# salesforce/LayoutDETR

Measured on AMD Instinct MI355X. Metric: images/sec G+D fwd-bwd, 256x256 bg x9 elems, higher is better.
Workload: dtype f32

## Files before the change

layoutdetr_amd/csrc/p3_engine.hip:

```cpp
#include <cstdlib>
#include "ldetr_common.hpp"
#include "../../include/ldetr_hip.h"

namespace ldetr {

bool splitk_ws_alloc(long tiles, size_t partial_bytes, float** ws, int** counters);
void note_engine_launch(bool bf16_split_pipe);

typedef unsigned u32x4 __attribute__((ext_vector_type(4)));
typedef __attribute__((address_space(3))) void lds_void;

struct P3Epi {
    float alpha;
    const float* col_scale;
    const float* col_bias;
    const char* res_p3;
    const float* res_f32;
    const char* mask_p3;
    int relu;
    char* out_p3;
    float* out_f32;
};

struct P3NtParams {
    const char* A;
    const char* B;
    unsigned a_bytes, b_bytes;
    int M, N, Cin;
    int KH, KW, stride, pad;
    int H, W, OH, OW;
    int out_H, out_W, out_step, out_py, out_px;
    int tap_mode;
    int kh0, kw0, tstep, nty, ntx;
    int nkt;
    int splitk;
    float* ws; int* ws_count;
    int mtiles, ntiles, xm, xn;
    int nclass, nimg;
    P3Epi ep;
    int ngroups;
};

struct P3Group2 {
    const char* A2; const char* B2;
    P3Epi ep2;
};

__device__ __forceinline__ float bf_lo(unsigned w) { return __uint_as_float(w << 16); }
__device__ __forceinline__ float bf_hi(unsigned w) { return __uint_as_float(w & 0xffff0000u); }

__device__ __forceinline__ bool xcd_tile(int b, int mtiles, int ntiles, int xm, int xn, int& tm, int& tn) {
    const int x = b & 7, i = b >> 3, xi = x / xn, xj = x - xi * xn;
    const int mlo = xi * mtiles / xm, mhi = (xi + 1) * mtiles / xm, nlo = xj * ntiles / xn, nhi = (xj + 1) * ntiles / xn;
    const int cn = nhi - nlo;
    if (cn <= 0 || i >= (mhi - mlo) * cn) return false;
    tm = mlo + i / cn; tn = nlo + i - (i / cn) * cn;
    return true;
}

template <int WM, int WN, int TM, int TN, typename RowMap>
__device__ __forceinline__ void p3_wave_epilogue(const P3Epi& ep, float* Cs, const f32x16 (&acc)[TM][TN], int lane, int nbase, int N, RowMap rowmap) {
    constexpr int CP = WN + 4;
    const int cl = lane & 31, kl = lane >> 5;
#pragma unroll
    for (int i = 0; i < TM; i++)
#pragma unroll
        for (int j = 0; j < TN; j++)
#pragma unroll
            for (int r = 0; r < 16; r++)
                Cs[(i * 32 + (r & 3) + 8 * (r >> 2) + 4 * kl) * CP + j * 32 + cl] = acc[i][j][r];
    constexpr int CH = WN / 8;
    constexpr int RPI = 64 / CH;
    const int ch = lane % CH, rl0 = lane / CH;
    const int n = nbase + ch * 8;
    float cs[8], cb[8];
#pragma unroll
    for (int e = 0; e < 8; e++) { cs[e] = ep.alpha; cb[e] = 0.f; }
    if (n < N) {
        if (ep.col_scale) {
            const float4 s0 = *reinterpret_cast<const float4*>(ep.col_scale + n), s1 = *reinterpret_cast<const float4*>(ep.col_scale + n + 4);
            cs[0] *= s0.x; cs[1] *= s0.y; cs[2] *= s0.z; cs[3] *= s0.w; cs[4] *= s1.x; cs[5] *= s1.y; cs[6] *= s1.z; cs[7] *= s1.w;
        }
        if (ep.col_bias) {
            const float4 s0 = *reinterpret_cast<const float4*>(ep.col_bias + n), s1 = *reinterpret_cast<const float4*>(ep.col_bias + n + 4);
            cb[0] = s0.x; cb[1] = s0.y; cb[2] = s0.z; cb[3] = s0.w; cb[4] = s1.x; cb[5] = s1.y; cb[6] = s1.z; cb[7] = s1.w;
        }
    }
#pragma unroll 2
    for (int it = 0; it < WM / RPI; it++) {
        const int rl = it * RPI + rl0;
        const long orow = rowmap(rl);
        if (orow < 0 || n >= N) continue;
        const float4 v0 = *reinterpret_cast<const float4*>(Cs + rl * CP + ch * 8), v1 = *reinterpret_cast<const float4*>(Cs + rl * CP + ch * 8 + 4);
        float v[8] = {v0.x, v0.y, v0.z, v0.w, v1.x, v1.y, v1.z, v1.w};
#pragma unroll
        for (int e = 0; e < 8; e++) v[e] = v[e] * cs[e] + cb[e];
        const long goff = (orow * N + n) * 6;
        if (ep.res_p3) {
            const u32x4 h = *reinterpret_cast<const u32x4*>(ep.res_p3 + goff), md = *reinterpret_cast<const u32x4*>(ep.res_p3 + goff + 16),
                        lo = *reinterpret_cast<const u32x4*>(ep.res_p3 + goff + 32);
#pragma unroll
            for (int e = 0; e < 4; e++) {
                v[2 * e] += bf_lo(h[e]) + (bf_lo(md[e]) + bf_lo(lo[e]));
                v[2 * e + 1] += bf_hi(h[e]) + (bf_hi(md[e]) + bf_hi(lo[e]));
            }
        }
        if (ep.res_f32) {
            const float4 r0 = *reinterpret_cast<const float4*>(ep.res_f32 + orow * N + n), r1 = *reinterpret_cast<const float4*>(ep.res_f32 + orow * N + n + 4);
            v[0] += r0.x; v[1] += r0.y; v[2] += r0.z; v[3] += r0.w; v[4] += r1.x; v[5] += r1.y; v[6] += r1.z; v[7] += r1.w;
        }
        if (ep.relu) {
#pragma unroll
            for (int e = 0; e < 8; e++) v[e] = v[e] < 0.f ? 0.f : v[e];
        }
        if (ep.mask_p3) {
            const u32x4 h = *reinterpret_cast<const u32x4*>(ep.mask_p3 + goff);
#pragma unroll
            for (int e = 0; e < 4; e++) {
                if ((h[e] << 16) - 1u >= 0x7f800000u) v[2 * e] = 0.f;
                if ((h[e] & 0xffff0000u) - 1u >= 0x7f800000u) v[2 * e + 1] = 0.f;
            }
        }
        if (ep.out_f32) {
            *reinterpret_cast<float4*>(ep.out_f32 + orow * N + n) = make_float4(v[0], v[1], v[2], v[3]);
            *reinterpret_cast<float4*>(ep.out_f32 + orow * N + n + 4) = make_float4(v[4], v[5], v[6], v[7]);
        }
        if (ep.out_p3) {
            u32x4 h, md, lo;
#pragma unroll
            for (int e = 0; e < 4; e++) { unsigned a, b, c; split2_bf16_exact(v[2 * e], v[2 * e + 1], a, b, c); h[e] = a; md[e] = b; lo[e] = c; }
            *reinterpret_cast<u32x4*>(ep.out_p3 + goff) = h;
            *reinterpret_cast<u32x4*>(ep.out_p3 + goff + 16) = md;
            *reinterpret_cast<u32x4*>(ep.out_p3 + goff + 32) = lo;
        }
    }
}

template <int TM, int TN, int NT>
__device__ __forceinline__ bool p3_splitk_reduce(f32x16 (&acc)[TM][TN], float* ws, int* ws_count, long tile, int ks, int splitk, int tile_elems, int tid, int* flag) {
    float* slot0 = ws + tile * splitk * (long)tile_elems;
    float* mine = slot0 + (long)ks * tile_elems;
#pragma unroll
    for (int i = 0; i < TM; i++)
#pragma unroll
        for (int j = 0; j < TN; j++)
#pragma unroll
            for (int r = 0; r < 16; r++)
                __hip_atomic_store(mine + ((i * TN + j) * 16 + r) * NT + tid, acc[i][j][r], __ATOMIC_RELAXED, __HIP_MEMORY_SCOPE_AGENT);
    asm volatile("s_waitcnt vmcnt(0)" ::: "memory");
    __syncthreads();
    if (tid == 0) {
        const int old = atomicAdd(ws_count + tile, 1);
        const int last = old == splitk - 1;
        if (last) __hip_atomic_store(ws_count + tile, 0, __ATOMIC_RELAXED, __HIP_MEMORY_SCOPE_AGENT);
        *flag = last;
    }
    __syncthreads();
    const int last = *flag;
    __syncthreads();
    if (!last) return false;
#pragma unroll
    for (int i = 0; i < TM; i++)
#pragma unroll
        for (int j = 0; j < TN; j++)
#pragma unroll
            for (int r = 0; r < 16; r++) acc[i][j][r] = 0.f;
    for (int sl = 0; sl < splitk; sl++) {
        const float* src = slot0 + (long)sl * tile_elems;
#pragma unroll
        for (int i = 0; i < TM; i++)
#pragma unroll
            for (int j = 0; j < TN; j++)
#pragma unroll
                for (int r = 0; r < 16; r++)
                    acc[i][j][r] += __hip_atomic_load(src + ((i * TN + j) * 16 + r) * NT + tid, __ATOMIC_RELAXED, __HIP_MEMORY_SCOPE_AGENT);
    }
    return true;
}

template <int TM, int TN>
__device__ __forceinline__ bool p3_acc_non_finite(const f32x16 (&acc)[TM][TN]) {
    float chk = 0.f;
#pragma unroll
    for (int i = 0; i < TM; i++)
#pragma unroll
        for (int j = 0; j < TN; j++)
#pragma unroll
            for (int r = 0; r < 16; r++) chk = fmaf(acc[i][j][r], 0.f, chk);
    return __builtin_amdgcn_ballot_w64(chk != chk) != 0ull;
}

typedef unsigned int ld128_t __attribute__((__vector_size__(16)));

__device__ __forceinline__ void p3_load_group(const __amdgpu_buffer_rsrc_t rs, unsigned vo, int so, float (&v)[8]) {
    const ld128_t h = __builtin_amdgcn_raw_buffer_load_b128(rs, vo, so, 0), md = __builtin_amdgcn_raw_buffer_load_b128(rs, vo, so + 16, 0),
                  lo = __builtin_amdgcn_raw_buffer_load_b128(rs, vo, so + 32, 0);
#pragma unroll
    for (int e = 0; e < 4; e++) {
        v[2 * e] = bf_lo(h[e]) + (bf_lo(md[e]) + bf_lo(lo[e]));
        v[2 * e + 1] = bf_hi(h[e]) + (bf_hi(md[e]) + bf_hi(lo[e]));
    }
}

__device__ __forceinline__ float p3_load_elem(const __amdgpu_buffer_rsrc_t rs, unsigned row, int c) {
    const unsigned vo = row == 0x80000000u ? row : row + (unsigned)((c >> 3) * 48 + (c & 7) * 2);
    const unsigned h = __builtin_amdgcn_raw_buffer_load_b16(rs, vo, 0, 0), md = __builtin_amdgcn_raw_buffer_load_b16(rs, vo, 16, 0),
                   lo = __builtin_amdgcn_raw_buffer_load_b16(rs, vo, 32, 0);
    return bf_lo(h) + (bf_lo(md) + bf_lo(lo));
}

template <int WM, int WN, int TM, int TN, typename Dot>
__device__ __forceinline__ void p3_cold_tile(f32x16 (&acc)[TM][TN], float* img, int lane, Dot dot) {
    for (int e = lane; e < WM * WN; e += 64) {
        const int row = e / WN, col = e - row * WN;
        const float v = dot(row, col);
        const int i = row >> 5, rr = row & 31, j = col >> 5, cl = col & 31;
// ... 139 lines not shown
    const int rr = lane >> 2, pq = (lane & 3) ^ ((rr >> 2) & 3);
    const int ktpt = p.Cin >> 5;
    unsigned offA[RGA], vmA[RGA], offB[RGB];
#pragma unroll
    for (int i = 0; i < RGA; i++) {
        unsigned vm, off;
        p3_nt_row(p, m0 + (w * RGA + i) * 16 + rr, off, vm);
        offA[i] = (ONE && vm == 0u) ? 0x80000000u : off + pq * 16; vmA[i] = vm;
    }
#pragma unroll
    for (int i = 0; i < RGB; i++) {
        const int n = n0 + (w * RGB + i) * 16 + rr;
        offB[i] = n < p.N ? (unsigned)n * (unsigned)(p.KH * p.KW * p.Cin) * 6u + pq * 16 : 0x80000000u;
    }

    int tap = ONE ? 0 : kt0 / ktpt, cc = kt0 - tap * ktpt;

    const int frr = cl & 15, frg = cl >> 4;
    unsigned fo[2][3];
#pragma unroll
    for (int s = 0; s < 2; s++)
#pragma unroll
        for (int pl = 0; pl < 3; pl++) {
            const int e = 3 * (2 * s + kl) + pl;
            fo[s][pl] = (unsigned)((frg * 3 + (e >> 2)) * 1024 + frr * 64 + (((e & 3) ^ ((frr >> 2) & 3)) << 4));
        }
    const unsigned foA = (unsigned)(wm * (WM / 16) * 3 * 1024), foB = (unsigned)(A_BYTES + wn * (WN / 16) * 3 * 1024);

    f32x16 acc[TM][TN];
#pragma unroll
    for (int i = 0; i < TM; i++)
#pragma unroll
        for (int j = 0; j < TN; j++)
#pragma unroll
            for (int r = 0; r < 16; r++) acc[i][j][r] = 0.f;

    const int nloc = kt1 - kt0;
    ld128_t ra[PF][RGA * 3], rb[PF][RGB * 3];
#pragma unroll
    for (int d = 0; d < PF; d++) p3_load_tile<BM, BN, NW, ONE>(p, rsA, rsB, offA, vmA, offB, tap, cc, ktpt, d < nloc, ra[d], rb[d]);
    if (nloc > 0) p3_store_tile<BM, BN, NW>(p3_smem, w, lane, ra[0], rb[0]);
    __syncthreads();
    for (int it0 = 0; it0 < nloc; it0 += PF) {
#pragma unroll
        for (int d = 0; d < PF; d++) {
            const int it = it0 + d;
            p3_load_tile<BM, BN, NW, ONE>(p, rsA, rsB, offA, vmA, offB, tap, cc, ktpt, it + PF < nloc, ra[d], rb[d]);
            __builtin_amdgcn_sched_barrier(0);
            if (it < nloc) {
                const char* sb = p3_smem + (it % NST) * ST_BYTES;
#pragma unroll
                for (int s = 0; s < 2; s++) {
                    bf16x8_t a[TM][3], b[TN][3];
#pragma unroll
                    for (int i = 0; i < TM; i++)
#pragma unroll
                        for (int pl = 0; pl < 3; pl++)
                            a[i][pl] = *reinterpret_cast<const bf16x8_t*>(sb + foA + i * (2 * 3 * 1024) + fo[s][pl]);
#pragma unroll
                    for (int j = 0; j < TN; j++)
#pragma unroll
                        for (int pl = 0; pl < 3; pl++)
                            b[j][pl] = *reinterpret_cast<const bf16x8_t*>(sb + foB + j * (2 * 3 * 1024) + fo[s][pl]);
#pragma unroll
                    for (int i = 0; i < TM; i++)
#pragma unroll
                        for (int j = 0; j < TN; j++) {
                            acc[i][j] = __builtin_amdgcn_mfma_f32_32x32x16_bf16(a[i][1], b[j][1], acc[i][j], 0, 0, 0);
                            acc[i][j] = __builtin_amdgcn_mfma_f32_32x32x16_bf16(a[i][0], b[j][2], acc[i][j], 0, 0, 0);
                            acc[i][j] = __builtin_amdgcn_mfma_f32_32x32x16_bf16(a[i][2], b[j][0], acc[i][j], 0, 0, 0);
                            acc[i][j] = __builtin_amdgcn_mfma_f32_32x32x16_bf16(a[i][0], b[j][1], acc[i][j], 0, 0, 0);
                            acc[i][j] = __builtin_amdgcn_mfma_f32_32x32x16_bf16(a[i][1], b[j][0], acc[i][j], 0, 0, 0);
                            acc[i][j] = __builtin_amdgcn_mfma_f32_32x32x16_bf16(a[i][0], b[j][0], acc[i][j], 0, 0, 0);
                        }
                }
                if (NST == 1) __syncthreads();
                if (it + 1 < nloc) p3_store_tile<BM, BN, NW>(p3_smem + ((it + 1) % NST) * ST_BYTES, w, lane, ra[(d + 1) % PF], rb[(d + 1) % PF]);
                __syncthreads();
            }
        }
    }

    constexpr int CP = WN + 4;
    if (p3_acc_non_finite<TM, TN>(acc)) {
        p3_cold_tile<WM, WN, TM, TN>(acc, reinterpret_cast<float*>(p3_smem) + w * (WM * CP), lane, [&](int row, int col) -> float {
            unsigned off, vm;
            p3_nt_row(p, m0 + wm * WM + row, off, vm);
            const int n = n0 + wn * WN + col;
            const unsigned ob = n < p.N ? (unsigned)n * (unsigned)(p.KH * p.KW * p.Cin) * 6u : 0x80000000u;
            float s = 0.f;
            for (int kt = kt0; kt < kt1; kt++) {
                const int tp = kt / ktpt;
                int sA, sB;
                p3_nt_koff(p, tp, kt - tp * ktpt, sA, sB);
                const unsigned vo = ((vm >> tp) & 1u) ? off : 0x80000000u;
                for (int g = 0; g < 4; g++) {
                    float a[8], b[8];
                    p3_load_group(rsA, vo, sA + g * 48, a); p3_load_group(rsB, ob, sB + g * 48, b);
#pragma unroll
                    for (int e = 0; e < 8; e++) s = fmaf(a[e], b[e], s);
                }
            }
            return s;
        });
    }
    if (p.splitk > 1 && !p3_splitk_reduce<TM, TN, NT>(acc, p.ws, p.ws_count, ws_tile0 + t, ks, p.splitk, BM * BN, tid, reinterpret_cast<int*>(p3_smem))) return;
    const int ohw = p.OH * p.OW;
    p3_wave_epilogue<WM, WN, TM, TN>(p.ep, reinterpret_cast<float*>(p3_smem) + w * (WM * CP), acc, lane, n0 + wn * WN, p.N, [&](int rl) -> long {
        const int m = m0 + wm * WM + rl;
        if (m >= p.M) return -1;
        if (p.out_step == 1 && p.out_H == p.OH && p.out_W == p.OW) return m;
        const int nn = m / ohw, rem = m - nn * ohw, oy = rem / p.OW, ox = rem - oy * p.OW;
        return ((long)nn * p.out_H + (oy * p.out_step + p.out_py)) * p.out_W + (ox * p.out_step + p.out_px);
    });
}

template <int BM, int BN, int NW, int PF, int NST, bool ONE = false>
__global__ __launch_bounds__(NW * 64) void p3_nt_kernel(P3NtParams p, P3Group2 g2) { p3_nt_body<BM, BN, NW, PF, NST, true, ONE>(p, g2, blockIdx.x, blockIdx.y, blockIdx.z); }

struct P3C3Params {
    const char* X; const char* Wt;
    unsigned x_bytes, w_bytes;
    int N_img, H, W, Cin, Nout;
    int lgPW, lgPH, NP;
    int HWp, HPIX, NH, NG;
    int ppr, ppi;
    int flip;
    int ncc;
    int splitk; float* ws; int* ws_count;
    int mtiles, ntiles, xm, xn;
    P3Epi ep;
    int ngroups;
};

constexpr int C3_NGMAX = 13, C3_A_BYTES = C3_NGMAX * 3072, C3_B_BYTES = 4 * 3072, C3_LDS = C3_A_BYTES + 3 * C3_B_BYTES;

__device__ __forceinline__ void p3_c3_decode_tile_row(const P3C3Params& p, int tm, int r, int& n, int& y0, int& x0, int& py, int& px) {
    const int lgpp = p.lgPW + p.lgPH;
    const int sp = r >> lgpp, q = r & ((1 << lgpp) - 1);
    py = q >> p.lgPW; px = q & ((1 << p.lgPW) - 1);
    const int pid = tm * p.NP + sp;
    n = pid / p.ppi; const int prem = pid - n * p.ppi;
    const int pr = prem / p.ppr, pc = prem - pr * p.ppr;
    y0 = pr << p.lgPH; x0 = pc << p.lgPW;
}

template <int TAP>
__device__ __forceinline__ void p3_c3_tap(const P3C3Params& p, const __amdgpu_buffer_rsrc_t rsA, const __amdgpu_buffer_rsrc_t rsB, char* smem, int w, int lane,
                                          const unsigned (&offA)[4], unsigned offB, int cc, bool more_cc, bool more_tile,
                                          ld128_t (&ar)[12], ld128_t (&br)[3], const unsigned (&h0)[2], const unsigned (&ce)[2][3], const unsigned (&fo)[2][3],
                                          unsigned foB, f32x16 (&acc)[2][1]) {
    if (more_tile) {
        const int ntap = TAP == 8 ? 0 : TAP + 1, ncc = TAP == 8 ? cc + 1 : cc;
        const int sB = ntap * p.Cin * 6 + ncc * 192;
#pragma unroll
        for (int j = 0; j < 3; j++) br[j] = __builtin_amdgcn_raw_buffer_load_b128(rsB, offB, sB + j * 64, 0);
    }
    if (more_cc) {
#pragma unroll
        for (int q = TAP * 12 / 9; q < (TAP + 1) * 12 / 9; q++)
            ar[q] = __builtin_amdgcn_raw_buffer_load_b128(rsA, offA[q / 3], (cc + 1) * 192 + (q % 3) * 64, 0);
    }
    constexpr int ty = TAP / 3, tx = TAP % 3;
    const int dt = p.flip ? (2 - ty) * p.HWp + (2 - tx) : ty * p.HWp + tx;
    unsigned hb[2], sw[2];
#pragma unroll
    for (int i = 0; i < 2; i++) {
        const unsigned h = h0[i] + dt;
        hb[i] = (h >> 4) * 3072 + ((h & 15) << 6);
        sw[i] = ((h >> 2) & 3) << 4;
    }
    const char* sb = smem + C3_A_BYTES + (TAP % 3) * C3_B_BYTES + foB;
#pragma unroll
    for (int s2 = 0; s2 < 2; s2++) {
        bf16x8_t a[2][3], b[3];
#pragma unroll
        for (int i = 0; i < 2; i++)
#pragma unroll
            for (int pl = 0; pl < 3; pl++) a[i][pl] = *reinterpret_cast<const bf16x8_t*>(smem + hb[i] + (ce[s2][pl] ^ sw[i]));
#pragma unroll
        for (int pl = 0; pl < 3; pl++) b[pl] = *reinterpret_cast<const bf16x8_t*>(sb + fo[s2][pl]);
#pragma unroll
        for (int i = 0; i < 2; i++) {
            acc[i][0] = __builtin_amdgcn_mfma_f32_32x32x16_bf16(a[i][1], b[1], acc[i][0], 0, 0, 0);
            acc[i][0] = __builtin_amdgcn_mfma_f32_32x32x16_bf16(a[i][0], b[2], acc[i][0], 0, 0, 0);
            acc[i][0] = __builtin_amdgcn_mfma_f32_32x32x16_bf16(a[i][2], b[0], acc[i][0], 0, 0, 0);
            acc[i][0] = __builtin_amdgcn_mfma_f32_32x32x16_bf16(a[i][0], b[1], acc[i][0], 0, 0, 0);
            acc[i][0] = __builtin_amdgcn_mfma_f32_32x32x16_bf16(a[i][1], b[0], acc[i][0], 0, 0, 0);
            acc[i][0] = __builtin_amdgcn_mfma_f32_32x32x16_bf16(a[i][0], b[0], acc[i][0], 0, 0, 0);
        }
    }
    if (more_tile) {
        char* dst = smem + C3_A_BYTES + ((TAP + 1) % 3) * C3_B_BYTES + w * 3072 + lane * 16;
#pragma unroll
        for (int j = 0; j < 3; j++) *reinterpret_cast<ld128_t*>(dst + j * 1024) = br[j];
    }
    __syncthreads();
}

template <bool GROUPS>
__device__ __forceinline__ void p3_c3_body(P3C3Params p, const P3Group2& g2, const int bx, const int by, const int bz) {
    constexpr int BM = 128, BN = 64, NT = 256, WM = 64, WN = 32;
    if (GROUPS && p.ngroups > 1 && bz > 0) { p.X = g2.A2; p.Wt = g2.B2; p.ep = g2.ep2; }
    extern __shared__ __attribute__((aligned(1024))) char p3_smem[];
    const int tid = threadIdx.x, lane = tid & 63, w = __builtin_amdgcn_readfirstlane(tid >> 6), wm = w >> 1, wn = w & 1;
    const int cl = lane & 31, kl = lane >> 5;
    int tm, tn;
    if (!xcd_tile(bx, p.mtiles, p.ntiles, p.xm, p.xn, tm, tn)) return;
    const int t = tm * p.ntiles + tn;
    const int n0 = tn * BN;
    const int ks = by;
    const int per = (p.ncc + p.splitk - 1) / p.splitk;
    const int cc0 = ks * per, cc1 = min(p.ncc, cc0 + per);

    const __amdgpu_buffer_rsrc_t rsA = __builtin_amdgcn_make_buffer_rsrc(const_cast<char*>(p.X), 0, p.x_bytes, 0x00020000);
    const __amdgpu_buffer_rsrc_t rsB = __builtin_amdgcn_make_buffer_rsrc(const_cast<char*>(p.Wt), 0, p.w_bytes, 0x00020000);

    const int rr = lane >> 2, pq = (lane & 3) ^ ((rr >> 2) & 3);
    unsigned offA[4], offB;
#pragma unroll
    for (int i = 0; i < 4; i++) {
        const int h = (w + 4 * i) * 16 + rr;
        unsigned off = 0x80000000u;
        if (h < p.NH) {
            const int sp = h / p.HPIX, rem = h - sp * p.HPIX, hy = rem / p.HWp, hx = rem - hy * p.HWp;
            const int pid = tm * p.NP + sp;
            const int n = pid / p.ppi, prem = pid - n * p.ppi, pr = prem / p.ppr, pc = prem - pr * p.ppr;
            const int y = (pr << p.lgPH) + hy - 1, x = (pc << p.lgPW) + hx - 1;
            if (n < p.N_img && y >= 0 && y < p.H && x >= 0 && x < p.W) off = (unsigned)(((n * p.H + y) * p.W + x) * p.Cin) * 6u + pq * 16;
        }
        offA[i] = off;
    }
    {
        const int n = n0 + w * 16 + rr;
        offB = n < p.Nout ? (unsigned)n * (unsigned)(9 * p.Cin) * 6u + pq * 16 : 0x80000000u;
    }
    unsigned h0[2];
#pragma unroll
    for (int i = 0; i < 2; i++) {
        const int r = wm * WM + i * 32 + cl;
        const int lgpp = p.lgPW + p.lgPH;
        const int sp = r >> lgpp, q = r & ((1 << lgpp) - 1);
        h0[i] = (unsigned)(sp * p.HPIX + (q >> p.lgPW) * p.HWp + (q & ((1 << p.lgPW) - 1)));
    }
    const int frr = cl & 15, frg = cl >> 4;
    unsigned ce[2][3], fo[2][3];
#pragma unroll
    for (int s2 = 0; s2 < 2; s2++)
#pragma unroll
        for (int pl = 0; pl < 3; pl++) {
            const int e = 3 * (2 * s2 + kl) + pl;
            ce[s2][pl] = (unsigned)(((e >> 2) * 1024) | ((e & 3) << 4));
            fo[s2][pl] = (unsigned)((frg * 3 + (e >> 2)) * 1024 + frr * 64 + (((e & 3) ^ ((frr >> 2) & 3)) << 4));
        }
    const unsigned foB = (unsigned)(wn * 2 * 3072);

    f32x16 acc[2][1];
#pragma unroll
    for (int i = 0; i < 2; i++)
#pragma unroll
        for (int r = 0; r < 16; r++) acc[i][0][r] = 0.f;

    ld128_t ar[12], br[3];
    if (cc1 > cc0) {
#pragma unroll
        for (int q = 0; q < 12; q++) ar[q] = __builtin_amdgcn_raw_buffer_load_b128(rsA, offA[q / 3], cc0 * 192 + (q % 3) * 64, 0);
#pragma unroll
        for (int j = 0; j < 3; j++) br[j] = __builtin_amdgcn_raw_buffer_load_b128(rsB, offB, cc0 * 192 + j * 64, 0);
#pragma unroll
        for (int q = 0; q < 12; q++)
            if (w + 4 * (q / 3) < C3_NGMAX) *reinterpret_cast<ld128_t*>(p3_smem + ((w + 4 * (q / 3)) * 3 + (q % 3)) * 1024 + lane * 16) = ar[q];
#pragma unroll
        for (int j = 0; j < 3; j++) *reinterpret_cast<ld128_t*>(p3_smem + C3_A_BYTES + w * 3072 + j * 1024 + lane * 16) = br[j];
    }
    __syncthreads();
    for (int cc = cc0; cc < cc1; cc++) {
        const bool more_cc = cc + 1 < cc1;
#define C3_TAP(T_) p3_c3_tap<T_>(p, rsA, rsB, p3_smem, w, lane, offA, offB, cc, more_cc, (T_) < 8 || more_cc, ar, br, h0, ce, fo, foB, acc)
        C3_TAP(0); C3_TAP(1); C3_TAP(2); C3_TAP(3); C3_TAP(4); C3_TAP(5); C3_TAP(6); C3_TAP(7); C3_TAP(8);
#undef C3_TAP
        if (more_cc) {
#pragma unroll
            for (int q = 0; q < 12; q++)
                if (w + 4 * (q / 3) < C3_NGMAX) *reinterpret_cast<ld128_t*>(p3_smem + ((w + 4 * (q / 3)) * 3 + (q % 3)) * 1024 + lane * 16) = ar[q];
            __syncthreads();
        }
    }

    constexpr int CP = WN + 4;
    static_assert(4 * WM * CP * 4 <= C3_LDS, "epilogue staging does not fit");
    if (p3_acc_non_finite<2, 1>(acc)) {
        p3_cold_tile<WM, WN, 2, 1>(acc, reinterpret_cast<float*>(p3_smem) + w * (WM * CP), lane, [&](int row, int col) -> float {
            int n, y0, x0, py, px;
            p3_c3_decode_tile_row(p, tm, wm * WM + row, n, y0, x0, py, px);
            if (n >= p.N_img) return 0.f;
            const int y = y0 + py, x = x0 + px, no = n0 + wn * WN + col;
            const unsigned ob = no < p.Nout ? (unsigned)no * (unsigned)(9 * p.Cin) * 6u : 0x80000000u;
            float s = 0.f;
            for (int cc = cc0; cc < cc1; cc++)
                for (int tap = 0; tap < 9; tap++) {
                    const int ty = tap / 3, tx = tap - ty * 3;
                    const int sy = y + (p.flip ? 1 - ty : ty - 1), sx = x + (p.flip ? 1 - tx : tx - 1);
                    const unsigned vo = (sy >= 0 && sy < p.H && sx >= 0 && sx < p.W) ? (unsigned)(((n * p.H + sy) * p.W + sx) * p.Cin) * 6u : 0x80000000u;
                    for (int g = 0; g < 4; g++) {
                        float a[8], b[8];
                        p3_load_group(rsA, vo, cc * 192 + g * 48, a); p3_load_group(rsB, ob, tap * p.Cin * 6 + cc * 192 + g * 48, b);
#pragma unroll
                        for (int e = 0; e < 8; e++) s = fmaf(a[e], b[e], s);
                    }
                }
            return s;
        });
    }
    if (p.splitk > 1 && !p3_splitk_reduce<2, 1, NT>(acc, p.ws, p.ws_count, t + bz * p.mtiles * p.ntiles, ks, p.splitk, BM * BN, tid, reinterpret_cast<int*>(p3_smem))) return;
    p3_wave_epilogue<WM, WN, 2, 1>(p.ep, reinterpret_cast<float*>(p3_smem) + w * (WM * CP), acc, lane, n0 + wn * WN, p.Nout, [&](int rl) -> long {
        int n, y0, x0, py, px;
        p3_c3_decode_tile_row(p, tm, wm * WM + rl, n, y0, x0, py, px);
        if (n >= p.N_img) return -1;
        return ((long)n * p.H + (y0 + py)) * p.W + (x0 + px);
    });
}

__global__ __launch_bounds__(256, 2) void p3_c3_kernel(P3C3Params p, P3Group2 g2) { p3_c3_body<true>(p, g2, blockIdx.x, blockIdx.y, blockIdx.z); }

struct P3TnParams {
    const char* dY; const char* X;
    unsigned dy_bytes, x_bytes;
    int Cout, Cin, KH, KW, stride, pad;
    int H, W, OH, OW;
    int npix;
    float inv_ohw, inv_ow;
    int mtiles, ntiles, splitk;
    const float* row_scale;
    float alpha;
    float* dW;
};

__device__ __forceinline__ void fastdivmod(int x, int d, float invd, int& q, int& r) {
    q = (int)((float)x * invd);
    r = x - q * d;
    if (r >= d) { ++q; r -= d; }
    if (r < 0) { --q; r += d; }
}

typedef unsigned u32x2_t __attribute__((ext_vector_type(2)));
__device__ __forceinline__ u32x2_t tr_read(unsigned addr) {
    u32x2_t v;
    asm volatile("ds_read_b64_tr_b16 %0, %1" : "=v"(v) : "v"(addr) : "memory");
    return v;
}
__device__ __forceinline__ void tr_wait() { asm volatile("s_waitcnt lgkmcnt(0)" ::: "memory"); __builtin_amdgcn_sched_barrier(0); }
__device__ __forceinline__ bf16x8_t tr_join(u32x2_t lo, u32x2_t hi) {
    const u32x4 v = {lo[0], lo[1], hi[0], hi[1]};
    return __builtin_bit_cast(bf16x8_t, v);
}

template <int BM, int BN>
__device__ __forceinline__ void p3_tn_load(const P3TnParams& p, const __amdgpu_buffer_rsrc_t rsA, const __amdgpu_buffer_rsrc_t rsB, int w, int lane,
                                           int k0, int kend, int m0, int n0, int kh, int kw, ld128_t* ra, ld128_t* rb) {
    constexpr int UA = BM / 64, UB = BN / 64;
    const int rg = w & 1, rr = lane >> 2, pq = (lane & 3) ^ ((rr >> 2) & 3);
    const int pix = k0 + rg * 16 + rr;
    const bool inr = pix < kend;
    const unsigned offA = inr ? (unsigned)pix * (unsigned)p.Cout * 6u + pq * 16 : 0x80000000u;
#pragma unroll
    for (int i = 0; i < UA; i++) {
        const int cb = (w >> 1) * UA + i;
        const int sA = (m0 + cb * 32) * 6;
#pragma unroll
        for (int j = 0; j < 3; j++) ra[i * 3 + j] = __builtin_amdgcn_raw_buffer_load_b128(rsA, offA, sA + j * 64, 0);
    }
    unsigned offB = 0x80000000u;
    {
        int n, rem, oy, ox;
        fastdivmod(pix, p.OH * p.OW, p.inv_ohw, n, rem);
        fastdivmod(rem, p.OW, p.inv_ow, oy, ox);
        const int sy = oy * p.stride - p.pad + kh, sx = ox * p.stride - p.pad + kw;
        if (inr && sy >= 0 && sy < p.H && sx >= 0 && sx < p.W)
            offB = (unsigned)(((n * p.H + oy * p.stride) * p.W + ox * p.stride) * p.Cin) * 6u + pq * 16;
    }
    const int sBt = (kh * p.W + kw) * p.Cin * 6;
#pragma unroll
    for (int i = 0; i < UB; i++) {
        const int cb = (w >> 1) * UB + i;
        const int sB = sBt + (n0 + cb * 32) * 6;
#pragma unroll
        for (int j = 0; j < 3; j++) rb[i * 3 + j] = __builtin_amdgcn_raw_buffer_load_b128(rsB, offB, sB + j * 64, 0);
    }
}

template <int BM, int BN>
__device__ __forceinline__ void p3_tn_store(char* sb, int w, int lane, const ld128_t* ra, const ld128_t* rb) {
    constexpr int UA = BM / 64, UB = BN / 64, A_BYTES = BM * 192;
    const int rg = w & 1;
#pragma unroll
    for (int i = 0; i < UA; i++)
#pragma unroll
        for (int j = 0; j < 3; j++) *reinterpret_cast<ld128_t*>(sb + ((((w >> 1) * UA + i) * 2 + rg) * 3 + j) * 1024 + lane * 16) = ra[i * 3 + j];
#pragma unroll
    for (int i = 0; i < UB; i++)
// ... 215 lines not shown
#pragma unroll
        for (int e = 0; e < 4; e++) { unsigned a, b, c; split2_bf16_exact(v[2 * e], v[2 * e + 1], a, b, c); h[e] = a; md[e] = b; lo[e] = c; }
        char* d = dst + u * 48;
        *reinterpret_cast<u32x4*>(d) = h; *reinterpret_cast<u32x4*>(d + 16) = md; *reinterpret_cast<u32x4*>(d + 32) = lo;
    }
}

__global__ __launch_bounds__(256) void p3_weight_prep_kernel(const long long* __restrict__ table, int nconv) {
    int c = 0;
    while (c + 1 < nconv && (long long)blockIdx.x >= table[(c + 1) * 8 + 7]) ++c;
    const long long* row = table + c * 8;
    const float* w = reinterpret_cast<const float*>(row[0]);
    const float* sc = reinterpret_cast<const float*>(row[1]);
    char* df = reinterpret_cast<char*>(row[2]);
    char* db = reinterpret_cast<char*>(row[3]);
    const int O = (int)row[4], T = (int)row[5], I = (int)row[6];
    const long u = ((long)blockIdx.x - row[7]) * 256 + threadIdx.x;
    const long units = (long)O * T * I / 8;
    if (u >= units) return;
    if (df) {
        const float4 v0 = *reinterpret_cast<const float4*>(w + u * 8), v1 = *reinterpret_cast<const float4*>(w + u * 8 + 4);
        const float v[8] = {v0.x, v0.y, v0.z, v0.w, v1.x, v1.y, v1.z, v1.w};
        u32x4 h, md, lo;
#pragma unroll
        for (int e = 0; e < 4; e++) { unsigned a, b, cc; split2_bf16_exact(v[2 * e], v[2 * e + 1], a, b, cc); h[e] = a; md[e] = b; lo[e] = cc; }
        char* d = df + u * 48;
        *reinterpret_cast<u32x4*>(d) = h; *reinterpret_cast<u32x4*>(d + 16) = md; *reinterpret_cast<u32x4*>(d + 32) = lo;
    }
    if (db) {
        const int i = (int)(u % I); const long r = u / I; const int tp = (int)(r % T); const int g = (int)(r / T);
        float v[8];
#pragma unroll
        for (int e = 0; e < 8; e++) v[e] = w[((long)(g * 8 + e) * T + tp) * I + i] * (sc ? sc[g * 8 + e] : 1.f);
        u32x4 h, md, lo;
#pragma unroll
        for (int e = 0; e < 4; e++) { unsigned a, b, cc; split2_bf16_exact(v[2 * e], v[2 * e + 1], a, b, cc); h[e] = a; md[e] = b; lo[e] = cc; }
        char* d = db + (((long)i * T + tp) * (O / 8) + g) * 48;
        *reinterpret_cast<u32x4*>(d) = h; *reinterpret_cast<u32x4*>(d + 16) = md; *reinterpret_cast<u32x4*>(d + 32) = lo;
    }
}

static void choose_xcd_array(int mtiles, int ntiles, double a_bytes, double b_bytes, int& xm, int& xn, long& grid_x) {
    double best = -1.0; xm = 8; xn = 1;
    for (int n = 1; n <= 8; n *= 2) {
        const int m = 8 / n;
        if ((n > ntiles && n > 1) || (m > mtiles && m > 1)) continue;
        const double cost = a_bytes * n + b_bytes * m;
        if (best < 0 || cost < best) { best = cost; xm = m; xn = n; }
    }
    grid_x = 8L * cdiv(mtiles, xm) * cdiv(ntiles, xn);
}


struct RaisedPerDevice { bool on[64] = {}; };
static bool raise_lds(const void* kern, size_t lds, const char* what, RaisedPerDevice& raised) {
    if (lds <= 64 * 1024) return true;
    int dev = 0;
    if (hipGetDevice(&dev) != hipSuccess || dev < 0 || dev >= 64) dev = -1;
    if (dev >= 0 && raised.on[dev]) return true;
    if (hipFuncSetAttribute(kern, hipFuncAttributeMaxDynamicSharedMemorySize, (int)lds) != hipSuccess) {
        set_error("%s: cannot raise the dynamic LDS limit to %zu bytes", what, lds);
        return false;
    }
    if (dev >= 0) raised.on[dev] = true;
    return true;
}

struct P3LastLaunch { int kind, bm, bn, nw, splitk, xm, xn, ncls, tn_splitk; long grid; };
static thread_local P3LastLaunch t_last = {0, 0, 0, 0, 0, 0, 0, 0, 0, 0};

struct NtGrid { long gx; int sk, ncls; size_t lds; };

template <int BM, int BN, int NW, int NST>
static NtGrid plan_nt(P3NtParams& p, int sk) {
    p.mtiles = cdiv(p.M, BM); p.ntiles = cdiv(p.N, BN);
    NtGrid g; g.ncls = p.nclass > 1 ? p.nclass : (p.ngroups > 1 ? p.ngroups : 1);
    const long nt = (long)p.mtiles * p.ntiles;
    choose_xcd_array(p.mtiles, p.ntiles, (double)p.M * p.Cin * 6.0, (double)p.N * p.KH * p.KW * p.Cin * 6.0, p.xm, p.xn, g.gx);
    if (sk > p.nkt) sk = p.nkt;
    if (sk < 1) sk = 1;
    p.splitk = sk; p.ws = nullptr; p.ws_count = nullptr;
    if (sk > 1 && !splitk_ws_alloc(nt * g.ncls, (size_t)nt * g.ncls * sk * BM * BN * sizeof(float), &p.ws, &p.ws_count)) p.splitk = sk = 1;
    g.sk = sk;
    constexpr int WGN_ = (NW == 8 && BN >= 128) ? 4 : 2, WM_ = BM / (NW / WGN_), WN_ = BN / WGN_;
    constexpr size_t lds_loop = (size_t)NST * (BM + BN) * 192, lds_epi = (size_t)NW * WM_ * (WN_ + 4) * 4;
    g.lds = lds_loop > lds_epi ? lds_loop : lds_epi;
    return g;
}

static long slot_target(double flops, long dflt) {
    static const double small = 1.5 * 1e9;
    return (flops < small && dflt > 256) ? 256 : dflt;
}
static double nt_flops(const P3NtParams& p) { return 2.0 * p.M * p.N * p.nkt * 32.0 * (p.nclass > 1 ? p.nclass : 1); }
static double tn_flops(const P3TnParams& p) { return 2.0 * p.npix * p.Cout * (double)p.Cin * p.KH * p.KW; }

static int nt_splitk(const P3NtParams& p, int bm, int bn, long slots) {
    const long nt = (long)cdiv(p.M, bm) * cdiv(p.N, bn);
    int sk = 1;
    if (nt < slots * 3 / 4) { sk = (int)(slots / nt); if (sk > p.nkt / 4) sk = p.nkt / 4; if (sk > 16) sk = 16; if (sk < 1) sk = 1; }
    return sk;
}

static bool nt_is_plain_gemm(const P3NtParams& p) { return p.KH * p.KW == 1 && p.pad == 0 && p.nclass <= 1 && (p.tap_mode == 0 || p.stride == 1); }

template <int BM, int BN, int NW, int PF, int NST>
static int launch_nt_cfg(P3NtParams& p, const P3Group2& g2, int sk, hipStream_t st) {
    const NtGrid g = plan_nt<BM, BN, NW, NST>(p, sk);
    if constexpr (PF == 1 && NST == 1 && (BM == BN) && (NW == 4 ? BM == 64 : BM == 128)) {
        if (nt_is_plain_gemm(p)) {
            auto kern1 = p3_nt_kernel<BM, BN, NW, PF, NST, true>;
            static RaisedPerDevice raised1;
            if (!raise_lds(reinterpret_cast<const void*>(kern1), g.lds, "p3_nt", raised1)) return LDETR_ERR_LAUNCH;
            hipLaunchKernelGGL(kern1, dim3((unsigned)g.gx, g.sk, g.ncls), NW * 64, g.lds, st, p, g2);
            t_last = {1, BM, BN, NW, g.sk, p.xm, p.xn, g.ncls, 0, g.gx};
            note_engine_launch(true);
            return check_launch("p3_nt");
        }
    }
    auto kern = p3_nt_kernel<BM, BN, NW, PF, NST>;
    static RaisedPerDevice raised;
    if (!raise_lds(reinterpret_cast<const void*>(kern), g.lds, "p3_nt", raised)) return LDETR_ERR_LAUNCH;
    hipLaunchKernelGGL(kern, dim3((unsigned)g.gx, g.sk, g.ncls), NW * 64, g.lds, st, p, g2);
    t_last = {1, BM, BN, NW, g.sk, p.xm, p.xn, g.ncls, 0, g.gx};
    note_engine_launch(true);
    return check_launch("p3_nt");
}

static int launch_nt(P3NtParams& p, const P3Group2& g2, bool forward, hipStream_t st) {
    static const int force_tile = (int)knob("P3_TILE", 0);
    int cfg = 3;
    if (forward && p.nclass <= 1 && ((p.M >= 65536 && p.N >= 128) || (p.M >= 16384 && p.N >= 256 && p.nkt <= 16))) cfg = 1;
    if (force_tile) cfg = force_tile;
    const int bm = cfg == 3 ? 64 : 128, bn = (cfg == 1 || cfg == 4) ? 128 : 64;
    const int sk = nt_splitk(p, bm, bn, slot_target(nt_flops(p), (cfg == 2 || cfg == 3) ? 512 : 256));
    switch (cfg) {
        case 1: return launch_nt_cfg<128, 128, 8, 1, 1>(p, g2, sk, st);
        case 2: return launch_nt_cfg<128, 64, 4, 1, 1>(p, g2, sk, st);
        case 3: return launch_nt_cfg<64, 64, 4, 1, 1>(p, g2, sk, st);
        default: return launch_nt_cfg<128, 128, 4, 1, 1>(p, g2, sk, st);
    }
}

static bool c3_geometry(int N, int H, int W, P3C3Params& p) {
    auto lg = [](int v) { int l = 0; while ((1 << l) < v) ++l; return (1 << l) == v ? l : -1; };
    int PW = W < 16 ? W : 16;
    if (lg(PW) < 0 || W % PW) return false;
    int PH = 128 / PW; if (PH > H) PH = H;
    while (PH > 1 && (H % PH || lg(PH) < 0)) PH >>= 1;
    if (lg(PH) < 0 || H % PH || 128 % (PW * PH)) return false;
    p.lgPW = lg(PW); p.lgPH = lg(PH); p.NP = 128 / (PW * PH);
    p.HWp = PW + 2; p.HPIX = (PH + 2) * (PW + 2); p.NH = p.NP * p.HPIX; p.NG = (p.NH + 15) / 16;
    if (p.NG > C3_NGMAX) return false;
    p.ppr = W / PW; p.ppi = (H / PH) * (W / PW);
    p.N_img = N; p.H = H; p.W = W;
    p.mtiles = (int)(((long)N * p.ppi + p.NP - 1) / p.NP);
    return true;
}

static long plan_c3(P3C3Params& p) {
    p.ntiles = cdiv(p.Nout, 64);
    const long nt = (long)p.mtiles * p.ntiles;
    int sk = 1;
    const long slots = slot_target(2.0 * p.N_img * p.H * p.W * (double)p.Nout * 9.0 * p.Cin, 512);
    if (nt < slots * 3 / 4) { sk = (int)(slots / nt); if (sk > p.ncc / 2) sk = p.ncc / 2; if (sk > 16) sk = 16; if (sk < 1) sk = 1; }
    if (sk > p.ncc) sk = p.ncc;
    p.splitk = sk; p.ws = nullptr; p.ws_count = nullptr;
    const int ng = p.ngroups > 1 ? p.ngroups : 1;
    if (sk > 1 && !splitk_ws_alloc(nt * ng, (size_t)nt * ng * sk * 128 * 64 * sizeof(float), &p.ws, &p.ws_count)) p.splitk = sk = 1;
// ... 275 lines not shown
```

Measured before the change: 494.9.

## Stage P3 epilogue output through LDS for coalesced row stores; prefetch residual loads

```diff
diff --git a/layoutdetr_amd/csrc/p3_engine.hip b/layoutdetr_amd/csrc/p3_engine.hip
--- a/layoutdetr_amd/csrc/p3_engine.hip
+++ b/layoutdetr_amd/csrc/p3_engine.hip
@@ -58,21 +58,29 @@
     return true;
 }
 
-template <int WM, int WN, int TM, int TN, typename RowMap>
-__device__ __forceinline__ void p3_wave_epilogue(const P3Epi& ep, float* Cs, const f32x16 (&acc)[TM][TN], int lane, int nbase, int N, RowMap rowmap) {
+template <int BM, int BN, int NW, int WGN>
+struct P3EpiLds {
+    static constexpr int WGM = NW / WGN, WM = BM / WGM, WN = BN / WGN, CP = WN + 4;
+    static constexpr int stage_bytes = NW * WM * CP * 4, image_bytes = BM * BN * 6;
+    static constexpr int main_bytes(int loop_bytes) { return loop_bytes > stage_bytes ? loop_bytes : stage_bytes; }
+    static constexpr int passes(int loop_bytes) { return image_bytes <= main_bytes(loop_bytes) ? 1 : 2; }
+    static constexpr int total_bytes(int loop_bytes) { return main_bytes(loop_bytes) + BM * 4; }
+};
+
+template <int BM, int BN, int NW, int WGN, int PASSES, typename RowMap>
+__device__ __forceinline__ void p3_block_epilogue(const P3Epi& ep, char* smem, int* rowtab, const f32x16 (&acc)[BM / (NW / WGN) / 32][BN / WGN / 32],
+                                                  int tid, int n0, int N, RowMap rowmap) {
+    constexpr int WGM = NW / WGN, WM = BM / WGM, WN = BN / WGN, TM = WM / 32, TN = WN / 32, NT = NW * 64;
     constexpr int CP = WN + 4;
+    const int lane = tid & 63, w = __builtin_amdgcn_readfirstlane(tid >> 6), wm = w / WGN, wn = w % WGN;
     const int cl = lane & 31, kl = lane >> 5;
-#pragma unroll
-    for (int i = 0; i < TM; i++)
-#pragma unroll
-        for (int j = 0; j < TN; j++)
-#pragma unroll
-            for (int r = 0; r < 16; r++)
-                Cs[(i * 32 + (r & 3) + 8 * (r >> 2) + 4 * kl) * CP + j * 32 + cl] = acc[i][j][r];
+    float* Cs = reinterpret_cast<float*>(smem) + w * (WM * CP);
     constexpr int CH = WN / 8;
     constexpr int RPI = 64 / CH;
+    constexpr int NIT = WM / RPI, IPP = NIT / PASSES;
+    static_assert(NIT % PASSES == 0, "image passes must divide the wave's row iterations");
     const int ch = lane % CH, rl0 = lane / CH;
-    const int n = nbase + ch * 8;
+    const int n = n0 + wn * WN + ch * 8;
     float cs[8], cb[8];
 #pragma unroll
     for (int e = 0; e < 8; e++) { cs[e] = ep.alpha; cb[e] = 0.f; }
@@ -86,19 +94,38 @@
             cb[0] = s0.x; cb[1] = s0.y; cb[2] = s0.z; cb[3] = s0.w; cb[4] = s1.x; cb[5] = s1.y; cb[6] = s1.z; cb[7] = s1.w;
         }
     }
-#pragma unroll 2
-    for (int it = 0; it < WM / RPI; it++) {
+    u32x4 ph[NIT], pm[NIT], pl[NIT];
+    u32x4 mk[NIT];
+    int orow[NIT];
+    bool live[NIT];
+#pragma unroll
+    for (int it = 0; it < NIT; it++) {
         const int rl = it * RPI + rl0;
-        const long orow = rowmap(rl);
-        if (orow < 0 || n >= N) continue;
+        orow[it] = (int)rowmap(wm * WM + rl);
+        if (ch == 0 && wn == 0) rowtab[wm * WM + rl] = orow[it];
+        live[it] = orow[it] >= 0 && n < N;
+    }
+    constexpr int HC = NIT > 2 ? 2 : NIT, NC = NIT / HC;
+    static_assert(NIT % HC == 0, "hoist chunks must divide the wave's row iterations");
+    auto issue = [&](int it) {
+        if (!live[it]) return;
+        const long goff = ((long)orow[it] * N + n) * 6;
+        if (ep.res_p3) {
+            ph[it] = *reinterpret_cast<const u32x4*>(ep.res_p3 + goff); pm[it] = *reinterpret_cast<const u32x4*>(ep.res_p3 + goff + 16);
+            pl[it] = *reinterpret_cast<const u32x4*>(ep.res_p3 + goff + 32);
+        }
+        if (ep.mask_p3) mk[it] = *reinterpret_cast<const u32x4*>(ep.mask_p3 + goff);
+    };
+    auto finish = [&](int it) {
+        if (!live[it]) return;
+        const int rl = it * RPI + rl0;
+        const long eoff = (long)orow[it] * N + n;
         const float4 v0 = *reinterpret_cast<const float4*>(Cs + rl * CP + ch * 8), v1 = *reinterpret_cast<const float4*>(Cs + rl * CP + ch * 8 + 4);
         float v[8] = {v0.x, v0.y, v0.z, v0.w, v1.x, v1.y, v1.z, v1.w};
 #pragma unroll
         for (int e = 0; e < 8; e++) v[e] = v[e] * cs[e] + cb[e];
-        const long goff = (orow * N + n) * 6;
         if (ep.res_p3) {
-            const u32x4 h = *reinterpret_cast<const u32x4*>(ep.res_p3 + goff), md = *reinterpret_cast<const u32x4*>(ep.res_p3 + goff + 16),
-                        lo = *reinterpret_cast<const u32x4*>(ep.res_p3 + goff + 32);
+            const u32x4 h = ph[it], md = pm[it], lo = pl[it];
 #pragma unroll
             for (int e = 0; e < 4; e++) {
                 v[2 * e] += bf_lo(h[e]) + (bf_lo(md[e]) + bf_lo(lo[e]));
@@ -106,7 +133,7 @@
             }
         }
         if (ep.res_f32) {
-            const float4 r0 = *reinterpret_cast<const float4*>(ep.res_f32 + orow * N + n), r1 = *reinterpret_cast<const float4*>(ep.res_f32 + orow * N + n + 4);
+            const float4 r0 = *reinterpret_cast<const float4*>(ep.res_f32 + eoff), r1 = *reinterpret_cast<const float4*>(ep.res_f32 + eoff + 4);
             v[0] += r0.x; v[1] += r0.y; v[2] += r0.z; v[3] += r0.w; v[4] += r1.x; v[5] += r1.y; v[6] += r1.z; v[7] += r1.w;
         }
         if (ep.relu) {
@@ -114,7 +141,7 @@
             for (int e = 0; e < 8; e++) v[e] = v[e] < 0.f ? 0.f : v[e];
         }
         if (ep.mask_p3) {
-            const u32x4 h = *reinterpret_cast<const u32x4*>(ep.mask_p3 + goff);
+            const u32x4 h = mk[it];
 #pragma unroll
             for (int e = 0; e < 4; e++) {
                 if ((h[e] << 16) - 1u >= 0x7f800000u) v[2 * e] = 0.f;
@@ -122,16 +149,56 @@
             }
         }
         if (ep.out_f32) {
-            *reinterpret_cast<float4*>(ep.out_f32 + orow * N + n) = make_float4(v[0], v[1], v[2], v[3]);
-            *reinterpret_cast<float4*>(ep.out_f32 + orow * N + n + 4) = make_float4(v[4], v[5], v[6], v[7]);
-        }
-        if (ep.out_p3) {
-            u32x4 h, md, lo;
-#pragma unroll
-            for (int e = 0; e < 4; e++) { unsigned a, b, c; split2_bf16_exact(v[2 * e], v[2 * e + 1], a, b, c); h[e] = a; md[e] = b; lo[e] = c; }
-            *reinterpret_cast<u32x4*>(ep.out_p3 + goff) = h;
-            *reinterpret_cast<u32x4*>(ep.out_p3 + goff + 16) = md;
-            *reinterpret_cast<u32x4*>(ep.out_p3 + goff + 32) = lo;
+            *reinterpret_cast<float4*>(ep.out_f32 + eoff) = make_float4(v[0], v[1], v[2], v[3]);
+            *reinterpret_cast<float4*>(ep.out_f32 + eoff + 4) = make_float4(v[4], v[5], v[6], v[7]);
+        }
+#pragma unroll
+        for (int e = 0; e < 4; e++) { unsigned a, b, c; split2_bf16_exact(v[2 * e], v[2 * e + 1], a, b, c); ph[it][e] = a; pm[it][e] = b; pl[it][e] = c; }
+    };
+#pragma unroll
+    for (int k = 0; k < HC; k++) issue(k);
+#pragma unroll
+    for (int i = 0; i < TM; i++)
+#pragma unroll
+        for (int j = 0; j < TN; j++)
+#pragma unroll
+            for (int r = 0; r < 16; r++)
+                Cs[(i * 32 + (r & 3) + 8 * (r >> 2) + 4 * kl) * CP + j * 32 + cl] = acc[i][j][r];
+#pragma unroll
+    for (int c = 0; c < NC; c++) {
+        if (c + 1 < NC) {
+#pragma unroll
+            for (int k = 0; k < HC; k++) issue((c + 1) * HC + k);
+        }
+#pragma unroll
+        for (int k = 0; k < HC; k++) finish(c * HC + k);
+    }
+    if (!ep.out_p3) return;
+    constexpr int ROWB = BN * 6, PPR = ROWB / 16, IMG_ROWS = WGM * IPP * RPI, PIECES = IMG_ROWS * PPR;
+    static_assert(PIECES % NT == 0 && IMG_ROWS * ROWB * PASSES == BM * BN * 6, "image pass geometry");
+    const int nb = (N - n0 < BN ? N - n0 : BN) * 6;
+    char* const obase = ep.out_p3 + (long)n0 * 6;
+#pragma unroll
+    for (int ps = 0; ps < PASSES; ps++) {
+        __syncthreads();
+#pragma unroll
+        for (int k = 0; k < IPP; k++) {
+            const int it = ps * IPP + k;
+            if (live[it]) {
+                char* dst = smem + (wm * (IPP * RPI) + k * RPI + rl0) * ROWB + (wn * CH + ch) * 48;
+                *reinterpret_cast<u32x4*>(dst) = ph[it];
+                *reinterpret_cast<u32x4*>(dst + 16) = pm[it];
+                *reinterpret_cast<u32x4*>(dst + 32) = pl[it];
+            }
+        }
+        __syncthreads();
+#pragma unroll
+        for (int q0 = 0; q0 < PIECES; q0 += NT) {
+            const int q = q0 + tid, ir = q / PPR, pc = q - ir * PPR;
+            const int wr = ir / (IPP * RPI), rest = ir - wr * (IPP * RPI);
+            const int orow = rowtab[wr * WM + ps * (IPP * RPI) + rest];
+            if (orow >= 0 && pc * 16 < nb)
+                *reinterpret_cast<u32x4*>(obase + (long)orow * N * 6 + pc * 16) = *reinterpret_cast<const u32x4*>(smem + q * 16);
         }
     }
 }
@@ -437,6 +504,7 @@
     }
 
     constexpr int CP = WN + 4;
+    using EL = P3EpiLds<BM, BN, NW, WGN>;
     if (p3_acc_non_finite<TM, TN>(acc)) {
         p3_cold_tile<WM, WN, TM, TN>(acc, reinterpret_cast<float*>(p3_smem) + w * (WM * CP), lane, [&](int row, int col) -> float {
             unsigned off, vm;
@@ -461,8 +529,8 @@
     }
     if (p.splitk > 1 && !p3_splitk_reduce<TM, TN, NT>(acc, p.ws, p.ws_count, ws_tile0 + t, ks, p.splitk, BM * BN, tid, reinterpret_cast<int*>(p3_smem))) return;
     const int ohw = p.OH * p.OW;
-    p3_wave_epilogue<WM, WN, TM, TN>(p.ep, reinterpret_cast<float*>(p3_smem) + w * (WM * CP), acc, lane, n0 + wn * WN, p.N, [&](int rl) -> long {
-        const int m = m0 + wm * WM + rl;
+    p3_block_epilogue<BM, BN, NW, WGN, EL::passes(NST * ST_BYTES)>(p.ep, p3_smem, reinterpret_cast<int*>(p3_smem + EL::main_bytes(NST * ST_BYTES)), acc, tid, n0, p.N, [&](int r) -> long {
+        const int m = m0 + r;
         if (m >= p.M) return -1;
         if (p.out_step == 1 && p.out_H == p.OH && p.out_W == p.OW) return m;
         const int nn = m / ohw, rem = m - nn * ohw, oy = rem / p.OW, ox = rem - oy * p.OW;
@@ -488,7 +556,8 @@
     int ngroups;
 };
 
-constexpr int C3_NGMAX = 13, C3_A_BYTES = C3_NGMAX * 3072, C3_B_BYTES = 4 * 3072, C3_LDS = C3_A_BYTES + 3 * C3_B_BYTES;
+constexpr int C3_NGMAX = 13, C3_A_BYTES = C3_NGMAX * 3072, C3_B_BYTES = 4 * 3072, C3_LOOP = C3_A_BYTES + 3 * C3_B_BYTES;
+constexpr int C3_LDS = P3EpiLds<128, 64, 4, 2>::total_bytes(C3_LOOP);
 
 __device__ __forceinline__ void p3_c3_decode_tile_row(const P3C3Params& p, int tm, int r, int& n, int& y0, int& x0, int& py, int& px) {
     const int lgpp = p.lgPW + p.lgPH;
@@ -643,7 +712,7 @@
     }
 
     constexpr int CP = WN + 4;
-    static_assert(4 * WM * CP * 4 <= C3_LDS, "epilogue staging does not fit");
+    static_assert(P3EpiLds<BM, BN, 4, 2>::main_bytes(C3_LOOP) == C3_LOOP && P3EpiLds<BM, BN, 4, 2>::passes(C3_LOOP) == 1, "epilogue staging / P3 image do not fit the k-loop's LDS");
     if (p3_acc_non_finite<2, 1>(acc)) {
         p3_cold_tile<WM, WN, 2, 1>(acc, reinterpret_cast<float*>(p3_smem) + w * (WM * CP), lane, [&](int row, int col) -> float {
             int n, y0, x0, py, px;
@@ -668,9 +737,9 @@
         });
     }
     if (p.splitk > 1 && !p3_splitk_reduce<2, 1, NT>(acc, p.ws, p.ws_count, t + bz * p.mtiles * p.ntiles, ks, p.splitk, BM * BN, tid, reinterpret_cast<int*>(p3_smem))) return;
-    p3_wave_epilogue<WM, WN, 2, 1>(p.ep, reinterpret_cast<float*>(p3_smem) + w * (WM * CP), acc, lane, n0 + wn * WN, p.Nout, [&](int rl) -> long {
+    p3_block_epilogue<BM, BN, 4, 2, 1>(p.ep, p3_smem, reinterpret_cast<int*>(p3_smem + C3_LOOP), acc, tid, n0, p.Nout, [&](int r) -> long {
         int n, y0, x0, py, px;
-        p3_c3_decode_tile_row(p, tm, wm * WM + rl, n, y0, x0, py, px);
+        p3_c3_decode_tile_row(p, tm, r, n, y0, x0, py, px);
         if (n >= p.N_img) return -1;
         return ((long)n * p.H + (y0 + py)) * p.W + (x0 + px);
     });
@@ -1052,9 +1121,8 @@
     p.splitk = sk; p.ws = nullptr; p.ws_count = nullptr;
     if (sk > 1 && !splitk_ws_alloc(nt * g.ncls, (size_t)nt * g.ncls * sk * BM * BN * sizeof(float), &p.ws, &p.ws_count)) p.splitk = sk = 1;
     g.sk = sk;
-    constexpr int WGN_ = (NW == 8 && BN >= 128) ? 4 : 2, WM_ = BM / (NW / WGN_), WN_ = BN / WGN_;
-    constexpr size_t lds_loop = (size_t)NST * (BM + BN) * 192, lds_epi = (size_t)NW * WM_ * (WN_ + 4) * 4;
-    g.lds = lds_loop > lds_epi ? lds_loop : lds_epi;
+    constexpr int WGN_ = (NW == 8 && BN >= 128) ? 4 : 2;
+    g.lds = (size_t)P3EpiLds<BM, BN, NW, WGN_>::total_bytes(NST * (BM + BN) * 192);
     return g;
 }
 
```

Result: no change. 497.6 (median of 6 runs) (+0.5%).
